# stevenknown/xpoly

Hardware: AMD Instinct MI355X
Metric: simplex pivots/sec (float tableau 4kx8k) (higher is better)
Workload: dtype f64; 1 GPU; dense LP m=4096 n=4095 (gen.hard_lp_f64: A~U(0.1,1), b=A x*, c=A^T y*), slack tableau 4096x8192 fp64 resident in HBM; one step = xpg_lp_begin (slack form rebuilt on the device) + 3840 pivots of the device-resident SIX::solveSlackForm loop = 120 full batches of 32; parallelism=replicas only (1 tableau per GPU)

## Files before the change

### xpoly_amd/csrc/ctx.hip.h

```cpp
#pragma once
#include <hip/hip_runtime.h>
#include <hip/hip_ext.h>
#include <map>
#include <mutex>
#include <string>
#include <utility>
#include <vector>
#include <stdio.h>
#include <stdlib.h>
#include <string.h>
#include "../../include/xpoly_amd.h"

namespace xpg { struct LoopState; }

struct xpg_ctx {
    int device;
    hipStream_t stream;
    std::string err;
    void * rowbuf; void * colbuf; xpg::LoopState * st; size_t row_cap, col_cap;
    void * stage; size_t stage_cap;
    void * hstage; size_t hstage_cap;
    void * hpack = 0; size_t hpack_cap = 0;
    void * hred = 0; size_t hred_cap = 0;
    std::vector<xpg_ctx *> lanes;
    std::vector<std::pair<void *, size_t> > dev_cache;
    size_t dev_cache_bytes = 0;
    void * slice_buf = 0; size_t slice_cap = 0;
    int loop_mode;
    int block_len;
    int loop_auto;
    int num_cus;
    int chain;
    int chain_local = 1;
    int chain_fold = 1;
    int chain_test_abort = 0;
    std::vector<hipEvent_t> ev0, ev1;
    int prof_cap, prof_n, prof_stride, prof_seen;
};

#define XPG_HIP(ctx, call)                                                         \
    do {                                                                           \
        hipError_t e_ = (call);                                                    \
        if (e_ != hipSuccess) {                                                    \
            (ctx)->err = std::string(#call) + ": " + hipGetErrorString(e_);        \
            return XPG_ERR_HIP;                                                    \
        }                                                                          \
    } while (0)

namespace xpg {

struct DeviceGuard {
    int prev = -1, mine = -1;
    explicit DeviceGuard(int device) : mine(device)
    {
        if (hipGetDevice(&prev) != hipSuccess) prev = -1;
        if (device >= 0 && prev != device) (void)hipSetDevice(device);
    }
    ~DeviceGuard() { if (prev >= 0 && mine >= 0 && prev != mine) (void)hipSetDevice(prev); }
    DeviceGuard(const DeviceGuard &) = delete;
    DeviceGuard & operator=(const DeviceGuard &) = delete;
};
#define XPG_BIND(ctx_) xpg::DeviceGuard xpg_bind_guard_((ctx_) ? (ctx_)->device : -1)

inline int round_up(int x, int a) { return (x + a - 1) / a * a; }

inline hipError_t lds_limit(const void * fn, int device, size_t bytes)
{
    static std::mutex mu;
    static std::map<std::pair<const void *, int>, size_t> cur;
    std::lock_guard<std::mutex> g(mu);
    size_t & c = cur[std::make_pair(fn, device)];
    if (bytes <= c) return hipSuccess;
    const hipError_t e = hipFuncSetAttribute(fn, hipFuncAttributeMaxDynamicSharedMemorySize, (int)bytes);
    if (e == hipSuccess) c = bytes;
    return e;
}

inline int pick_ld(int W)
{
    int ld = W % 16 == 0 ? W : round_up(W, 64);
    if (ld % 4112 == 0 || (ld + 16) % 4096 == 0) ld += 16;
    return ld;
}

struct DevBuf {
    void * p; size_t cap; xpg_ctx * owner;
    DevBuf() : p(0), cap(0), owner(0) {}
// ... 60 lines not shown
```

### xpoly_amd/csrc/lp_chain.hip.h

```cpp
#pragma once
#include "lp_blocked.hip.h"

namespace xpg {

enum { ST_CHAIN_STUCK = XPG_ERR_CHAIN_STUCK, CH_SPIN_LIMIT = 1 << 21, CH_CLOSE = 0x7FFFFFFF,
       CH_ARRIVE_TICKS = 30000,
       CH_VETO_TICKS = 100000,
       CH_GO = 1, CH_ABORT = 2 };
typedef unsigned int ch_u32x4 __attribute__((ext_vector_type(4)));

__device__ __forceinline__ unsigned long long ch_lo64(ch_u32x4 g) { return ((unsigned long long)g.y << 32) | g.x; }

__device__ __forceinline__ void ch_load_record(const void * p, ch_u32x4 (&g)[6])
{
    asm volatile("global_load_dwordx4 %0, %6, off sc1\n\t"
                 "global_load_dwordx4 %1, %6, off offset:16 sc1\n\t"
                 "global_load_dwordx4 %2, %6, off offset:32 sc1\n\t"
                 "global_load_dwordx4 %3, %6, off offset:48 sc1\n\t"
                 "global_load_dwordx4 %4, %6, off offset:64 sc1\n\t"
                 "global_load_dwordx4 %5, %6, off offset:80 sc1\n\t"
                 "s_waitcnt vmcnt(0)"
                 : "=&v"(g[0]), "=&v"(g[1]), "=&v"(g[2]), "=&v"(g[3]), "=&v"(g[4]), "=&v"(g[5]) : "v"(p) : "memory");
}
__device__ __forceinline__ void ch_load4(const void * p0, const void * p1, const void * p2, const void * p3,
// ... 110 lines not shown
{
    const unsigned lo = (unsigned)dpp_row_shr<CTRL>((int)(unsigned)x), hi = (unsigned)dpp_row_shr<CTRL>((int)(unsigned)(x >> 32));
    const unsigned long long t = ((unsigned long long)hi << 32) | lo;
    return t < x ? t : x;
}
__device__ __forceinline__ unsigned long long ch_wave_min_u64(unsigned long long x)
{
    x = ch_min_step<0x111>(x); x = ch_min_step<0x112>(x); x = ch_min_step<0x114>(x); x = ch_min_step<0x118>(x);
    const unsigned long long a = ch_readlane_u64(x, 15), b = ch_readlane_u64(x, 31), c = ch_readlane_u64(x, 47), d = ch_readlane_u64(x, 63);
    const unsigned long long ab = a < b ? a : b, cd = c < d ? c : d;
    return ab < cd ? ab : cd;
}

enum { CH_NAP_FROM = 96 };
#ifndef CH_POLL_NAP
#define CH_POLL_NAP 1
#endif
#ifndef CH_NAP_PICK
#define CH_NAP_PICK 32
#endif
#ifndef CH_NAP_PREP
#define CH_NAP_PREP 32
#endif

struct ChHist { double h[BLK_MAX]; };
__device__ __forceinline__ void ch_hist_load(ChHist & H, const double * hist)
{
#pragma unroll
    for (int s = 0; s < BLK_MAX; s++) H.h[s] = hist[64 * s];
}
template <bool STAR> __device__ __forceinline__ double ch_replay(double start, const ChHist & H, double cv, int t, int star)
{
    double a = start;
#pragma unroll
    for (int s = 0; s < BLK_MAX; s += 4) {
        if (s >= t) break;
        double p0 = H.h[s] * ch_readlane_f64(cv, s), p1 = H.h[s + 1] * ch_readlane_f64(cv, s + 1);
        double p2 = H.h[s + 2] * ch_readlane_f64(cv, s + 2), p3 = H.h[s + 3] * ch_readlane_f64(cv, s + 3);
        if (STAR) {
            const double ident = -0.0;
            p0 = s > star ? p0 : ident; p1 = s + 1 > star ? p1 : ident; p2 = s + 2 > star ? p2 : ident; p3 = s + 3 > star ? p3 : ident;
        }
        a = a + p0; a = a + p1; a = a + p2; a = a + p3;
    }
    return a;
}

struct ChWinner { int r, enter, leave, qstar, cc; uint32_t w; double a; unsigned long long cnv; };
enum { CH_CLOSE_ROW = 0x7FFFFFFE, CH_UNORDERED_ROW = 0x7FFFFFFD };

__device__ __forceinline__ char * ch_rec_g0(const LpView<F64> & v, int w) { return (char *)(v.blkR + BLK_REC_G0) + (size_t)w * 16; }
__device__ __forceinline__ char * ch_rec_pay(const LpView<F64> & v, int w) { return (char *)(v.blkR + BLK_REC_PAY) + (size_t)w * (BLK_REC_PAY_WORDS * 8); }
__device__ __forceinline__ char * ch_part_g0(const LpView<F64> & v, int w) { return (char *)v.blkP + (size_t)w * 16; }
__device__ __forceinline__ char * ch_part_pay(const LpView<F64> & v, int w) { return (char *)(v.blkP + BLK_PART_PAY) + (size_t)w * (BLK_PART_PAY_INTS * 4); }

__device__ __forceinline__ int ch_poll_records(const LpView<F64> & v, int npick, unsigned tag, int lane, ChWinner & W)
{
    const int nu = (npick + 63) >> 6;
    const int k0 = lane, k1 = lane + 64, k2 = lane + 128, k3 = lane + 192;
    const void * p0 = ch_rec_g0(v, k0 < npick ? k0 : k0 % npick);
    const void * p1 = ch_rec_g0(v, k1 < npick ? k1 : k0 % npick);
    const void * p2 = ch_rec_g0(v, k2 < npick ? k2 : k0 % npick);
    const void * p3 = ch_rec_g0(v, k3 < npick ? k3 : k0 % npick);
    ch_u32x4 g0, g1, g2, g3;
    unsigned spins = 0;
    for (;;) {
        bool ok;
        if (nu == 1) { g0 = ch_load1(p0); ok = g0.w == tag; }
        else { ch_load4(p0, p1, p2, p3, g0, g1, g2, g3); ok = g0.w == tag && g1.w == tag && g2.w == tag && g3.w == tag; }
        if (__all(ok)) break;
        if (++spins > CH_SPIN_LIMIT) return -3;
        __builtin_amdgcn_s_sleep(CH_POLL_NAP);
    }
    unsigned long long key = ~0ull; int row = INT_MAX, rec = 0;
    if (k0 < npick) { key = ch_lo64(g0); row = (int)g0.z; rec = k0; }
    if (nu > 1) {
        if (k1 < npick && ch_lo64(g1) < key) { key = ch_lo64(g1); row = (int)g1.z; rec = k1; }
        if (k2 < npick && ch_lo64(g2) < key) { key = ch_lo64(g2); row = (int)g2.z; rec = k2; }
        if (k3 < npick && ch_lo64(g3) < key) { key = ch_lo64(g3); row = (int)g3.z; rec = k3; }
    }
    if (__builtin_amdgcn_readfirstlane((int)g0.z) == CH_CLOSE_ROW) return -1;
    const unsigned long long kmin = ch_wave_min_u64(key);
    if (kmin == 0ull) return -1;
    if (kmin == ~0ull) return -2;
    const int myrow = key == kmin ? row : INT_MAX;
    W.r = wave_min_int(myrow);
    const unsigned long long hit = __ballot(myrow == W.r);
    return __builtin_amdgcn_readlane(rec, __ffsll((long long)hit) - 1);
}
__device__ __forceinline__ bool ch_load_winner(const LpView<F64> & v, int widx, unsigned tag, ChWinner & W)
{
    const char * p = ch_rec_pay(v, widx);
    ch_u32x4 g1, g2, g3;
    unsigned spins = 0;
    for (;;) {
        ch_load3(p, p + 16, p + 32, g1, g2, g3);
        if (__all(g1.w == tag && g2.w == tag && g3.w == tag)) break;
        if (++spins > CH_SPIN_LIMIT) return false;
        __builtin_amdgcn_s_sleep(CH_POLL_NAP);
    }
    W.a = __builtin_bit_cast(double, ch_lo64(g1)); W.leave = (int)g1.z;
    W.w = g2.x; W.cc = (int)g2.y; W.enter = (int)(g2.z & 0xFFFFFFu); W.qstar = (int)(g2.z >> 24) - 1;
    W.cnv = ch_lo64(g3);
    return true;
}

template <bool LOCAL> __device__ __forceinline__ void ch_commit_loop(const LpView<F64> & v, int batch, int t0, int B, int npick, int nprep,
                                                                     unsigned budget, unsigned done, unsigned tp, bool fold_next)
{
    LoopState * st = v.st;
    const int lane = (int)threadIdx.x;
    for (int t = t0; t < B; t++) {
        const unsigned tag = blk_epoch(batch, t);
        ChWinner g;
        const int widx = ch_poll_records(v, npick, tag, lane, g);
        if (widx == -3 || (widx >= 0 && !ch_load_winner(v, widx, tag, g))) { if (lane == 0) ch_st(&st->status, (int)ST_CHAIN_STUCK); return; }
        if (widx < 0) {
            if (lane == 0 && (widx == -2 || budget != 0)) st->blk.closed = 1;
            if (lane == 0 && t == 0) {
                st->blk.batch = batch; st->blk.n = 0; st->blk.closed = 1; st->blk.generic = 0;
                if (widx == -2) st->blk.want_generic = 1;
            }
            ch_drain();
            if (lane == 0)
                ch_store_granule<LOCAL>(ch_part_g0(v, nprep), (unsigned long long)(unsigned)INT_MAX, ((unsigned long long)(unsigned)CH_CLOSE_ROW << 32) | (unsigned long long)tag);
            return;
        }
        if (lane == 0) {
            const int enter = g.enter, leave = g.leave, r = g.r;
            if (!((g.w >> (leave & 31)) & 1u)) {
                ch_stl<LOCAL>(&v.ppt[(size_t)enter * v.pw + (leave >> 5)], g.w | (1u << (leave & 31)));
                if (LOCAL) ch_st_plain(&v.rowcnt[enter], ch_ld(&v.rowcnt[enter]) + 1);
                else __hip_atomic_fetch_add(&v.rowcnt[enter], 1, __ATOMIC_RELAXED, __HIP_MEMORY_SCOPE_AGENT);
                ch_stl<LOCAL>(&v.colcnt[leave], g.cc + 1);
            }
            ch_stl<LOCAL>(&v.nv[enter], (uint8_t)0); ch_stl<LOCAL>(&v.nv[leave], (uint8_t)1);
            ch_stl<LOCAL>(&v.bv[enter], (uint8_t)1); ch_stl<LOCAL>(&v.bv[leave], (uint8_t)0);
            ch_stl<LOCAL>(&v.eq2bv[r], enter); ch_stl<LOCAL>(&v.bv2eq[enter], r); ch_stl<LOCAL>(&v.bv2eq[leave], -1);
            if ((int)tp < v.trace_cap) { v.trace[2 * tp] = enter; v.trace[2 * tp + 1] = leave; }
            st->total_pivots = tp + 1;
            st->done = done + 1;
            st->blk.budget = budget - 1;
            if (t == 0) { st->blk.batch = batch; st->blk.closed = 0; st->blk.generic = 0; }
            st->blk.r[t] = r; st->blk.n = t + 1;
            st->blk.la_from_state = 0;
            st->blk.la_epoch = tag;
            if (t == B - 1 && fold_next) {
                for (int x = 0; x < 8; x++) st->blk.ch_arrive[x] = 0u;
                st->blk.ch_decide = 0u;
                st->blk.ch0_la_epoch = tag; st->blk.ch0_budget = budget - 1; st->blk.ch0_done = done + 1; st->blk.ch0_tp = tp + 1;
                st->blk.ch0_ticket = blk_ticket0(batch + 1);
            }
        }
        ch_drain();
        if (lane == 0)
            ch_store_granule<LOCAL>(ch_part_g0(v, nprep), (unsigned long long)(unsigned)INT_MAX, ((unsigned long long)(unsigned)g.r << 32) | (unsigned long long)tag);
        tp += 1; done += 1; budget -= 1;
    }
}

#ifdef XPG_STAMPS
__device__ unsigned long long g_ch_ts[4][BLK_MAX][8];
#define CH_TS(pt_) do { if (lane == 0 && tsw >= 0) g_ch_ts[tsw][t][pt_] = wall_clock64(); } while (0)
#else
#define CH_TS(pt_) do { } while (0)
#endif

inline int ch_hist_slots(int B, int line) { return line ? (B + 3) / 4 * 4 : BLK_MAX; }
inline size_t ch_lds_bytes(int B, int line)
{
    const size_t plain = (size_t)BLK_MAX * 64 * 8, with_line = (size_t)ch_hist_slots(B, line) * 64 * 8 + (size_t)line * 64 * 8;
    return line ? (with_line > plain ? with_line : plain) : plain;
}
template <bool LOCAL, int LINE>
__global__ __launch_bounds__(64) void k_blk_chain(LpView<F64> v, int batch, int t0, int B, int npick, int nprep, int nparts0, int force_abort, int fold_next)
{
    extern __shared__ __attribute__((aligned(16))) double ch_hist[];
    if (LOCAL && (blockIdx.x & 7u)) return;
    LoopState * st = v.st;
    const int w = LOCAL ? (int)(blockIdx.x >> 3) : (int)blockIdx.x, lane = (int)threadIdx.x;
    const unsigned nworkers = LOCAL ? gridDim.x >> 3 : gridDim.x;
    const bool fold = t0 == 0;
    if ((fold ? st->blk.ch0_ticket != blk_ticket0(batch) : st->blk.ch_epoch != blk_epoch(batch, t0 - 1)) ||
        st->status != ST_RUNNING || st->pricing != 0 || (fold && (st->blk.la_from_state != 0 || st->blk.want_generic != 0))) return;
    unsigned budget = fold ? st->blk.ch0_budget : st->blk.ch_budget, done = fold ? st->blk.ch0_done : st->blk.ch_done;
    const unsigned tp0 = fold ? st->blk.ch0_tp : st->blk.ch_tp;
    const unsigned la_tag = st->blk.ch0_la_epoch;
    const unsigned max_iter = st->max_iter;
    char * const decision = ch_part_g0(v, BLK_DECISION_SLOT);
    const unsigned roll_tag = fold ? blk_ticket0(batch) : blk_epoch(batch, t0 - 1);
    if (lane == 0) __hip_atomic_fetch_add(&st->blk.ch_arrive[LOCAL ? ch_xcc_id() : 0], 1u, __ATOMIC_RELAXED, __HIP_MEMORY_SCOPE_AGENT);
    if (w == (int)nworkers - 1) {
        const unsigned long long t_in = wall_clock64();
        bool go = false, misplaced = false;
        for (;;) {
#ifdef XPG_TEST_HOOKS
            if (force_abort) { misplaced = force_abort == 2; break; }
#endif
            const unsigned mine = ch_ld(&st->blk.ch_arrive[lane & 7]);
            unsigned sum = 0, top = 0;
#pragma unroll
            for (int x = 0; x < 8; x++) { const unsigned c = (unsigned)__builtin_amdgcn_readlane((int)mine, x); sum += c; top = c > top ? c : top; }
            if (top >= nworkers) { go = true; break; }
            if (sum >= nworkers) { misplaced = true; break; }
            if (wall_clock64() - t_in > (unsigned long long)CH_ARRIVE_TICKS) break;
            __builtin_amdgcn_s_sleep(CH_POLL_NAP);
        }
        unsigned prev = 0u;
        if (lane == 0) prev = atomicCAS(&st->blk.ch_decide, 0u, go ? (unsigned)CH_GO : (unsigned)CH_ABORT);
        prev = (unsigned)__builtin_amdgcn_readfirstlane((int)prev);
        if (prev != 0u) return;
        if (lane == 0) {
            if (go) { st->blk.ch_runs += 1u; if (fold) st->blk.ch_folds += 1u; }
            else { st->blk.closed = 1; st->blk.ch_aborts += 1u; if (misplaced) st->blk.ch_misplaced += 1u; }
        }
        ch_drain();
        if (lane == 0) ch_store_granule<false>(decision, (unsigned long long)(go ? CH_GO : CH_ABORT), (unsigned long long)roll_tag);
        if (go) ch_commit_loop<LOCAL>(v, batch, t0, B, npick, nprep, budget, done, tp0, fold_next != 0);
        return;
    }
    const int m = v.m, W = v.W, rhs = v.rhs, ld = v.ld, lim = v.rhs - 1;
    const bool picker = w < npick;
    const double * __restrict__ tab = (const double *)v.tab;
    double * K = (double *)v.blkK;
    double * E = (double *)v.blkE;
    double * const hist = ch_hist + lane;
    const int hslots = LINE ? (B + 3) / 4 * 4 : BLK_MAX;
    bool decided = false;
// ... 1 lines not shown
        if (decided) return true;
        unsigned spins = 0;
        const unsigned long long t_wait = wall_clock64();
        bool asked = false;
        for (;;) {
            const ch_u32x4 g = ch_load1(decision);
            if (g.z == roll_tag) { if (g.x != (unsigned)CH_GO) return false; decided = true; return true; }
            if (!asked && wall_clock64() - t_wait > (unsigned long long)CH_VETO_TICKS) {
                asked = true;
                unsigned prev = 0u;
                if (lane == 0) prev = atomicCAS(&st->blk.ch_decide, 0u, (unsigned)CH_ABORT);
                prev = (unsigned)__builtin_amdgcn_readfirstlane((int)prev);
                if (prev == 0u) {
                    if (lane == 0) { st->blk.closed = 1; st->blk.ch_aborts += 1u; }
                    ch_drain();
                    if (lane == 0) ch_store_granule<false>(decision, (unsigned long long)CH_ABORT, (unsigned long long)roll_tag);
                    return false;
                }
                if (prev == (unsigned)CH_ABORT) return false;
            }
            if (++spins > CH_SPIN_LIMIT) { if (lane == 0) ch_st(&st->status, (int)ST_CHAIN_STUCK); return false; }
            __builtin_amdgcn_s_sleep(CH_POLL_NAP);
        }
    };
#ifdef XPG_STAMPS
    const int tsw = w == 0 ? 0 : (w == npick - 1 ? 1 : (w == npick ? 2 : (w == npick + nprep - 1 ? 3 : -1)));
#endif

    const bool crowded = npick + nprep > CH_NAP_FROM;
    if (picker) {
        const int i = w * 64 + lane;
        const bool has_row = i < m;
        const int ic = has_row ? i : 0;
        for (int s = 0; s < hslots; s++) hist[64 * s] = 0.0;
        for (int s = 0; s < t0; s++) hist[64 * s] = has_row ? K[(size_t)ic * BLK_MAX + s] : 0.0;
        double * const lcache = ch_hist + (size_t)hslots * 64 + lane;
        int line_group = -1;
        int bi = v.eq2bv[ic];
        int sstar = -1;
        double bcur = tab[(size_t)ic * ld + rhs];
        double klast = 0.0;
        for (int s = 0; s < t0; s++) {
            const int rs = st->blk.r[s];
            if (rs == i) sstar = s;
            const double ks = has_row ? K[(size_t)ic * BLK_MAX + s] : 0.0;
            if (s + 1 < t0) {
                const double eb = E[(size_t)s * ld + rhs];
                const double pb = ks * eb;
                bcur = (rs == i) ? eb : (bcur + pb);
            } else klast = ks;
        }
        int r_prev = t0 > 0 ? st->blk.r[t0 - 1] : -1;
        int first_prev = -1;
#pragma unroll 1
        for (int t = t0; t < B; t++) {
            const unsigned want_part = t > 0 ? blk_epoch(batch, t - 1) : la_tag, tag = blk_epoch(batch, t);
            CH_TS(0);
            ChHist H;
            ch_hist_load(H, hist);
            if (CH_NAP_PICK && crowded && t > t0) __builtin_amdgcn_s_sleep(CH_NAP_PICK);
            const int cnt = t == t0 ? nparts0 : nprep;
            const int lo = t == t0 ? 1 : 0;
            int nf = INT_MAX;
            for (int base = 0; base <= cnt; base += 256) {
                const int span = cnt + 1 - base;
                auto slot = [&](int k) -> const void * {
                    int kk = k <= cnt ? k : base + (lane % span);
                    kk = kk < lo ? lo : kk;
                    return ch_part_g0(v, kk == 0 ? nprep : kk - 1);
                };
                const void * p0 = slot(base + lane);
                const void * p1 = slot(base + lane + 64);
                const void * p2 = slot(base + lane + 128);
                const void * p3 = slot(base + lane + 192);
                ch_u32x4 g0, g1, g2, g3;
                unsigned spins = 0;
                for (;;) {
                    ch_load4(p0, p1, p2, p3, g0, g1, g2, g3);
                    const bool ok = g0.z == want_part && g1.z == want_part && g2.z == want_part && g3.z == want_part;
                    if (__all(ok)) break;
                    if (base == 0 && lo == 0 && (unsigned)__builtin_amdgcn_readfirstlane((int)g0.z) == want_part
                        && __builtin_amdgcn_readfirstlane((int)g0.w) == CH_CLOSE_ROW) return;
                    if (++spins > CH_SPIN_LIMIT) { if (lane == 0) ch_st(&st->status, (int)ST_CHAIN_STUCK); return; }
                    __builtin_amdgcn_s_sleep(CH_POLL_NAP);
                }
                nf = min(min(nf, (int)g0.x), min(min((int)g1.x, (int)g2.x), (int)g3.x));
                if (base == 0 && lo == 0) {
                    r_prev = __builtin_amdgcn_readfirstlane((int)g0.w);
                    if (r_prev == CH_CLOSE_ROW) return;
                    if (i == r_prev) { bi = first_prev; sstar = t - 1; }
                }
            }
            CH_TS(1);
            const int first = wave_min_int(nf);
            const bool fast = first >= 0 && first < rhs && done < max_iter && budget != 0;
            if (!fast) {
                if (!wait_decision()) return;
                if (lane == 0) ch_store_granule3<LOCAL>(ch_rec_g0(v, w), ~0u, ~0u, (unsigned)CH_CLOSE_ROW, tag);
                return;
            }
            double x0_mem = 0.0;
            constexpr int LN = LINE ? LINE : 16;
            double2 lnew[LN / 2];
            const bool line_miss = LINE && first / LN != line_group;
            if (!LINE) x0_mem = tab[(size_t)ic * ld + first];
            else if (line_miss) {
                const double2 * lp2 = (const double2 *)&tab[(size_t)ic * ld + (size_t)(first / LN) * LN];
#pragma unroll
                for (int q = 0; q < LN / 2; q++) lnew[q] = lp2[q];
            }
            const uint32_t pw_word = ch_ld(&v.ppt[(size_t)first * v.pw + (bi >> 5)]);
            const int cc = ch_ld(&v.colcnt[bi]);
            const double ev_mem = ch_ld(&E[(size_t)(lane + 1 < t ? lane : 0) * ld + first]);
            const double c0_mem = v.obj[first].v;
            double ev = 0.0;
            if (t == 0) {
                if (lane == 33) ev = c0_mem;
            } else {
                const bool fresh = lane >= 32 && lane <= 34;
                const char * gp = ch_part_pay(v, (lane == 34 ? rhs : first) >> 6) + (fresh ? 16 * (lane - 32) : 0);
                unsigned spins = 0;
                for (;;) {
                    const ch_u32x4 g = ch_load1(gp);
                    if (__all(g.z == want_part || !fresh)) { if (fresh) ev = __builtin_bit_cast(double, ch_lo64(g)); break; }
                    if (++spins > CH_SPIN_LIMIT) { if (lane == 0) ch_st(&st->status, (int)ST_CHAIN_STUCK); return; }
                    __builtin_amdgcn_s_sleep(CH_POLL_NAP);
                }
            }
            CH_TS(2);
            if (lane + 1 < t) ev = ev_mem;
            if (LINE && line_miss) {
#pragma unroll
                for (int q = 0; q < LN / 2; q++) { lcache[64 * (2 * q)] = lnew[q].x; lcache[64 * (2 * q + 1)] = lnew[q].y; }
                line_group = first / LN;
            }
            const double x0 = LINE ? lcache[64 * (first % LN)] : x0_mem;
            const double ec_new = ch_readlane_f64(ev, 32), eb_new = ch_readlane_f64(ev, 34);
            const unsigned long long cnv_bits = __builtin_bit_cast(unsigned long long, ch_readlane_f64(ev, 33));
            if (lane == t - 1) ev = ec_new;
            if (lane >= t) ev = -1.0;
            if (t > 0) {
                const double pb = klast * eb_new;
                bcur = (i == r_prev) ? eb_new : (bcur + pb);
            }
            double a;
            if (__any(sstar >= 0)) {
                const double es = __shfl(ev, sstar >= 0 ? sstar : 0);
                a = ch_replay<true>(sstar >= 0 ? es : x0, H, ev, t, sstar);
            } else a = ch_replay<false>(x0, H, ev, t, -1);
            CH_TS(5);
            klast = -a;
            hist[64 * t] = klast;
            if (!wait_decision()) return;
            if (has_row) ch_stl<LOCAL>(&K[(size_t)i * BLK_MAX + t], klast);
            unsigned long long key = ~0ull;
            bool unordered = false;
            if (has_row && !le(F64(a), zero<F64>()) && !((pw_word >> (bi & 31)) & 1u) && cc < lim) {
                const double q = bcur / a;
                unordered = q != q;
                key = ch_ratio_key(q);
            }
            if (__any(unordered)) {
                if (lane == 0) ch_store_granule3<LOCAL>(ch_rec_g0(v, w), 0u, 0u, (unsigned)CH_UNORDERED_ROW, tag);
                key = ~0ull;
            }
            const bool told = __any(unordered);
            CH_TS(6);
            const unsigned long long kmin = ch_wave_min_u64(key);
            const unsigned long long hit = __ballot(key == kmin);
            const bool publisher = kmin != ~0ull ? (lane == __ffsll((long long)hit) - 1) : (lane == 0);
            CH_TS(7);
            if (publisher && !told) {
                ch_store_granule3<LOCAL>(ch_rec_g0(v, w), (unsigned)kmin, (unsigned)(kmin >> 32), (unsigned)(kmin != ~0ull ? i : INT_MAX), tag);
                const unsigned long long ab = to_bits(F64(a));
                char * pay = ch_rec_pay(v, w);
                ch_store_granule3<LOCAL>(pay, (unsigned)ab, (unsigned)(ab >> 32), (unsigned)bi, tag);
                ch_store_granule3<LOCAL>(pay + 16, pw_word, (unsigned)cc, (unsigned)first | ((unsigned)(sstar + 1) << 24), tag);
                ch_store_granule3<LOCAL>(pay + 32, (unsigned)cnv_bits, (unsigned)(cnv_bits >> 32), 0u, tag);
            }
            CH_TS(3);
            first_prev = first;
            done += 1; budget -= 1;
        }
        return;
    }

    const int wp = w - npick;
    const int j = wp * 64 + lane;
    const bool has_col = j < W;
    const int jc = has_col ? j : 0;
    for (int s = 0; s < hslots; s++) hist[64 * s] = 0.0;
    for (int s = 0; s < t0; s++) hist[64 * s] = has_col ? E[(size_t)s * ld + jc] : 0.0;
    F64 oj = has_col ? v.obj[jc] : zero<F64>();
    if (!wait_decision()) return;
#pragma unroll 1
    for (int t = t0; t < B; t++) {
        const unsigned tag = blk_epoch(batch, t);
        CH_TS(0);
        ChHist H;
        ch_hist_load(H, hist);
        if (CH_NAP_PREP && crowded && t > t0) __builtin_amdgcn_s_sleep(CH_NAP_PREP);
        ChWinner g;
        const int widx = ch_poll_records(v, npick, tag, lane, g);
        if (widx == -3) { if (lane == 0) ch_st(&st->status, (int)ST_CHAIN_STUCK); return; }
        if (widx < 0) return;
        CH_TS(4);
        const int r = g.r;
        const double x0 = tab[(size_t)r * ld + jc];
        const bool in_vars = has_col && j < rhs;
        const int nv_mem = (int)ch_ld(&v.nv[in_vars ? jc : 0]), rc_mem = ch_ld(&v.rowcnt[in_vars ? jc : 0]);
        const double kv_mem = ch_ld(&K[(size_t)r * BLK_MAX + (lane < t ? lane : 0)]);
        if (!ch_load_winner(v, widx, tag, g)) { if (lane == 0) ch_st(&st->status, (int)ST_CHAIN_STUCK); return; }
        const int nvj = in_vars ? nv_mem : 0, rcj0 = in_vars ? rc_mem : INT_MAX;
        const double kv = lane < t ? kv_mem : -1.0;
        CH_TS(1);
        const int enter = g.enter, leave = g.leave;
        const F64 sc = div(one<F64>(), F64(g.a));
        const int smode = scale_mode(sc);
        const F64 cnv = from_bits<F64>(g.cnv);
        const int cmode = scale_mode(cnv);
        const int qstar = __builtin_amdgcn_readfirstlane(g.qstar);
        const double x = qstar >= 0 ? ch_replay<true>(hist[64 * qstar], H, kv, t, qstar) : ch_replay<false>(x0, H, kv, t, -1);
        CH_TS(2);
        const F64 e = scaled(F64(x), sc, smode);
        hist[64 * t] = e.v;
        CH_TS(5);
        int nf = INT_MAX, any = 0;
        if (has_col) {
            ch_stl<LOCAL>(&E[(size_t)t * ld + j], e.v);
            F64 tt = mul(e, minus_one<F64>());
            if (j >= rhs) tt = neg(tt);
            tt = scaled(tt, cnv, cmode);
            const bool in = j < rhs;
            const bool nv_mem = in && j != enter && j != leave && nvj != 0;
            const bool nv_old = in && (j == enter ? true : (j == leave ? false : nv_mem));
            const bool nv_new = in && (j == enter ? false : (j == leave ? true : nv_mem));
            const int rcj = (in && j != enter) ? rcj0 : INT_MAX;
            if (j < enter && in && !nv_old) oj = zero<F64>();
            oj = add(tt, oj);
            v.obj[j] = oj;
            if (nv_new && gt(oj, zero<F64>())) { any = 1; if (rcj < lim) nf = j; }
        }
        CH_TS(3);
        nf = wave_min_int(nf);
        any = __ballot(any != 0) != 0ull ? 1 : 0;
        char * pay = ch_part_pay(v, wp);
        if (has_col && j == nf) {
            ch_store_granule<LOCAL>(pay, to_bits(e), (unsigned long long)tag);
            ch_store_granule<LOCAL>(pay + 16, to_bits(oj), (unsigned long long)tag);
        }
        if (has_col && j == rhs) ch_store_granule<LOCAL>(pay + 32, to_bits(e), (unsigned long long)tag);
        if (lane == 0) ch_store_granule<LOCAL>(ch_part_g0(v, wp), ((unsigned long long)(unsigned)any << 32) | (unsigned)nf, (unsigned long long)tag);
        CH_TS(6);
    }
}

}
```

### xpoly_amd/csrc/lp_host.hip.h

```cpp
#pragma once
#include <hip/hip_runtime.h>
#include <hip/hip_ext.h>
#include <map>
#include <mutex>
#include <string>
#include <type_traits>
#include <utility>
#include <vector>
#include <stdio.h>
#include "../../include/xpoly_amd.h"
#include "ctx.hip.h"
#include "lp_kernels.hip.h"
#include "lp_blocked.hip.h"
#include "lp_chain.hip.h"

namespace xpg {

template <class S> inline void launch_update(xpg_ctx * ctx, const LpView<S> & v, int guarded);
inline bool prof_open(xpg_ctx * ctx)
{
    if (ctx->prof_n >= ctx->prof_cap) return false;
    if ((ctx->prof_seen++ % ctx->prof_stride) != 0) return false;
    (void)hipEventRecord(ctx->ev0[ctx->prof_n], ctx->stream);
    return true;
// ... 46 lines not shown
inline bool blk_shape_ok(int W) { return (W + 255) / 256 <= 510; }
inline bool chain_shape_ok(const xpg_ctx * ctx, int m, int W)
{
    const int cpick = (m + 63) / 64, cprep = (W + 63) / 64;
    const int cus = ctx->num_cus > 0 ? ctx->num_cus : 1;
    return cpick <= BLK_REC_MAX && cprep <= 510 && cpick + cprep + 1 <= 8 * cus;
}
struct BlkPlan {
    bool chain;
    bool local;
    int line;
    int cpick, cprep, workers;
    size_t lds;
    int sweep_rows;
};
inline BlkPlan blk_plan(const xpg_ctx * ctx, int m, int W, int ld, int B, bool ref_pricing, bool chain_off, bool chain_spread, bool fold)
{
    BlkPlan p;
    p.cpick = (m + 63) / 64; p.cprep = (W + 63) / 64; p.workers = p.cpick + p.cprep + 1;
    const int cus = ctx->num_cus > 0 ? ctx->num_cus : 1;
    p.chain = ctx->chain && !chain_off && ref_pricing && (B > 1 || fold) && chain_shape_ok(ctx, m, W);
    p.local = p.chain && ctx->chain_local && !chain_spread && p.workers <= (cus / 8) * 9;
    static const int line_env = [] { const char * s = xpg_hook("XPG_CHAIN_LINE"); return s ? atoi(s) : -1; }();
    auto line_fits = [&](int cols) {
        return (size_t)p.workers * ch_lds_bytes(B, cols) <= (size_t)(cus / 8) * 160 * 1024 &&
               (size_t)p.workers <= (size_t)(cus / 8) * ((size_t)160 * 1024 / ch_lds_bytes(B, cols));
    };
    const bool want_line = p.local && (line_env == 1 || line_env == 8 || (line_env != 0 && ld % 512 == 0));
    p.line = !want_line ? 0 : (line_env != 8 && line_fits(16)) ? 16 : line_fits(8) ? 8 : 0;
    p.lds = ch_lds_bytes(B, p.line);
    p.sweep_rows = (size_t)m * ld * sizeof(double) > ((size_t)320 << 20) ? 32 : 16;
    return p;
}
template <class S> inline void launch_blk_batch(xpg_ctx *, const LpView<S> &, int, int, bool, bool, bool, bool, bool, bool) {}
template <> inline void launch_blk_batch<F64>(xpg_ctx * ctx, const LpView<F64> & v, int batch, int B, bool ref_pricing, bool closes_often, bool chain_off,
                                              bool chain_spread, bool fold, bool next_folds)
{
    const int strips = (v.W + 511) / 512;
    const int tq = (v.W + 63) / 64 <= 510 ? 64 : 256, tp = 64;
    const int want_pick = (v.m + tp - 1) / tp;
    const int npick = want_pick < BLK_PICK_WGS ? want_pick : BLK_PICK_WGS;
    const dim3 gprep((v.W + tq - 1) / tq);
    const BlkPlan pl = blk_plan(ctx, v.m, v.W, v.ld, B, ref_pricing, chain_off, chain_spread, fold);
    const int cpick = pl.cpick, cprep = pl.cprep, workers = pl.workers;
    for (int t = 0; t < B; t++) {
        if (pl.chain && (t == 1 || fold)) {
            const int t0 = fold ? 0 : 1;
            const int test_abort = ctx->chain_test_abort;
            const bool local = pl.local;
            const int fa = test_abort > 0 ? (batch % test_abort == test_abort - 1 ? 1 : 0)
                                          : (test_abort < 0 && local && batch % -test_abort == -test_abort - 1 ? 2 : 0);
            const int nparts0 = (int)gprep.x;
            const int fn = next_folds ? 1 : 0;
            const int line = pl.line;
            const size_t lds = pl.lds;
            if (local && line == 16) hipLaunchKernelGGL((k_blk_chain<true, 16>), dim3(8 * workers), dim3(64), lds, ctx->stream, v, batch, t0, B, cpick, cprep, nparts0, fa, fn);
            else if (local && line == 8) hipLaunchKernelGGL((k_blk_chain<true, 8>), dim3(8 * workers), dim3(64), lds, ctx->stream, v, batch, t0, B, cpick, cprep, nparts0, fa, fn);
            else if (local) hipLaunchKernelGGL((k_blk_chain<true, 0>), dim3(8 * workers), dim3(64), lds, ctx->stream, v, batch, t0, B, cpick, cprep, nparts0, fa, fn);
            else hipLaunchKernelGGL((k_blk_chain<false, 0>), dim3(workers), dim3(64), lds, ctx->stream, v, batch, t0, B, cpick, cprep, nparts0, fa, fn);
            break;
        }
        hipLaunchKernelGGL(k_blk_pick, dim3(npick), dim3(tp), 0, ctx->stream, v, batch, t, (int)gprep.x);
        if (t == 0) hipLaunchKernelGGL(k_blk_pick_generic, dim3(1), dim3(1024), 0, ctx->stream, v, batch, (int)gprep.x);
        hipLaunchKernelGGL(k_blk_prep, gprep, dim3(tq), 0, ctx->stream, v, batch, t);
    }
    const bool timed = B == ctx->block_len && ctx->prof_n < ctx->prof_cap && (ctx->prof_seen++ % ctx->prof_stride) == 0;
    hipEvent_t e0 = timed ? ctx->ev0[ctx->prof_n] : nullptr, e1 = timed ? ctx->ev1[ctx->prof_n] : nullptr;
#define XPG_BLK_LAUNCH(ROWS_, UNR_, CAP_)                                                                                 \
    hipExtLaunchKernelGGL((k_blk_sweep<ROWS_, UNR_, CAP_>), dim3(strips, (v.m + ROWS_ - 1) / ROWS_), dim3(256), 0,        \
                          ctx->stream, e0, e1, 0, (double *)v.tab, v.m, v.W, v.ld, (const double *)v.blkE,                \
                          (const double *)v.blkK, v.st, batch, 0, ctx->block_len)
#define XPG_BLK_FULL(ROWS_, UNR_, NB_)                                                                                    \
    hipExtLaunchKernelGGL((k_blk_sweep_full<ROWS_, UNR_, NB_>), dim3(blk_sweep_grid(strips, (v.m + ROWS_ - 1) / ROWS_)), \
                          dim3(256), 0, ctx->stream, e0, e1, 0, (double *)v.tab, v.m, v.W, v.ld,                          \
                          (const double *)v.blkE, (const double *)v.blkK, v.st, batch, closes_often ? 1 : 0,              \
                          batch & 1, ctx->block_len)
    const bool full = B == 32 || B == 24 || B == 16;
    if (B == 32 && pl.sweep_rows == 32) XPG_BLK_FULL(32, 2, 32);
    else if (B == 32) XPG_BLK_FULL(16, 2, 32);
    else if (B == 24) XPG_BLK_FULL(16, 2, 24);
    else if (B == 16) XPG_BLK_FULL(16, 4, 16);
    else if (B <= 8) XPG_BLK_LAUNCH(32, 8, 8);
    else XPG_BLK_LAUNCH(32, 4, 16);
    if (closes_often && full)
        hipLaunchKernelGGL((k_blk_sweep<32, 4, 16>), dim3(strips, (v.m + 31) / 32), dim3(256), 0, ctx->stream, (double *)v.tab,
                           v.m, v.W, v.ld, (const double *)v.blkE, (const double *)v.blkK, v.st, batch, B, ctx->block_len);
#undef XPG_BLK_LAUNCH
#undef XPG_BLK_FULL
    if (timed) ctx->prof_n++;
}
template <> inline void launch_update<R32>(xpg_ctx * ctx, const LpView<R32> & v, int guarded)
{
    const bool timed = prof_open(ctx);
    hipLaunchKernelGGL((k_update_r32<1>), dim3(v.m, (v.W + 255) / 256), dim3(256), 0, ctx->stream, v, guarded);
    if (timed) prof_close(ctx);
}

struct LpBase {
    virtual ~LpBase() {}
    xpg_ctx * ctx;
    int kind;
};

template <class S> struct Lp : LpBase {
    LpView<S> v;
    int n0;
    int m;
    S * d_leq; S * d_tgtf;
    S * d_maxv;
    std::vector<void *> owned;
    size_t tab_elems;
    int ld_cap = 0;
// ... 397 lines not shown
```

### xpoly_amd/csrc/xpoly_amd.hip

```cpp
#include <hip/hip_runtime.h>
#include <stdlib.h>
#include <string.h>
#include <atomic>
#include <new>
#include <map>
#include <algorithm>
#include <thread>
#include <vector>
#include "../../include/xpoly_amd.h"
#ifndef XPG_PART
#define XPG_PART (-1)
#endif
#define XPG_IN(p_) (XPG_PART < 0 || XPG_PART == (p_))
#include "scalar.hip.h"
#include "ctx.hip.h"
#if XPG_IN(0)
#include "lp_kernels.hip.h"
#include "lp_pipe_r32.hip.h"
#include "lp_fused_r32.hip.h"
#include "lp_host.hip.h"
#include "warm_mip.hip.h"
#include "warm_mip_batch.hip.h"
#endif
#if XPG_IN(1) || XPG_IN(2)
// ... 13 lines not shown
namespace xpg {
extern template int batch_dev<F64>(xpg_ctx *, int, int, const F64 *, const F64 *, int, int, unsigned, int32_t *, F64 *, F64 *, uint32_t *, int);
extern template int batch_dev<R32>(xpg_ctx *, int, int, const R32 *, const R32 *, int, int, unsigned, int32_t *, R32 *, R32 *, uint32_t *, int);
}
#elif XPG_PART == 1
namespace xpg {
template int batch_dev<F64>(xpg_ctx *, int, int, const F64 *, const F64 *, int, int, unsigned, int32_t *, F64 *, F64 *, uint32_t *, int);
template int batch_dev<R32>(xpg_ctx *, int, int, const R32 *, const R32 *, int, int, unsigned, int32_t *, R32 *, R32 *, uint32_t *, int);
}
#endif

static_assert(sizeof(F64) == 8 && sizeof(R32) == 8, "both scalars are 8 bytes");
static_assert(sizeof(xpg_rat32) == sizeof(R32), "ABI layout of a rational");

#if XPG_IN(0)
struct xpg_lp { LpBase * impl; };

extern "C" {

const char * xpg_version(void) { return "xpoly_amd 0.1 (gfx950)"; }

int xpg_device_count(void)
{
    int n = 0;
    if (hipGetDeviceCount(&n) != hipSuccess) return 0;
    return n;
}

int xpg_create(xpg_ctx ** out, int device)
{
    if (!out) return XPG_ERR_SHAPE;
    *out = 0;
    int n = 0;
    if (hipGetDeviceCount(&n) != hipSuccess || n <= 0 || device < 0 || device >= n)
        return XPG_ERR_NO_DEVICE;
    xpg::DeviceGuard bind(device);
    xpg_ctx * c = new (std::nothrow) xpg_ctx();
    if (!c) return XPG_ERR_ALLOC;
    c->device = device;
    c->rowbuf = c->colbuf = 0; c->st = 0; c->row_cap = c->col_cap = 0;
    c->stage = 0; c->stage_cap = 0;
    c->hstage = 0; c->hstage_cap = 0;
    const char * lm = xpg_env("XPG_LOOP");
    if (lm && lm[0] == 's') lm = nullptr;
    c->loop_mode = lm && lm[0] == 'b' ? 3 : 0;
    const char * ch = xpg_env("XPG_CHAIN");
    c->chain = ch ? atoi(ch) : 1;
    const char * cx = xpg_hook("XPG_CHAIN_XCD");
    c->chain_local = cx ? (atoi(cx) != 0 ? 1 : 0) : 1;
    const char * cf = xpg_hook("XPG_CHAIN_FOLD");
    c->chain_fold = cf ? (atoi(cf) != 0 ? 1 : 0) : 1;
    const char * cta = xpg_hook("XPG_CHAIN_TEST_ABORT");
    c->chain_test_abort = cta ? atoi(cta) : 0;
    c->num_cus = 0;
    if (hipDeviceGetAttribute(&c->num_cus, hipDeviceAttributeMultiprocessorCount, device) != hipSuccess) c->num_cus = 0;
    c->loop_auto = lm ? 0 : 1;
    const char * bl = xpg_env("XPG_BLOCK");
    c->block_len = bl ? atoi(bl) : BLK_DEFAULT;
    if (c->block_len < 1) c->block_len = 1;
    if (c->block_len > BLK_MAX) c->block_len = BLK_MAX;
    c->prof_cap = 0; c->prof_n = 0; c->prof_stride = 1; c->prof_seen = 0;
    if (hipStreamCreateWithFlags(&c->stream, hipStreamNonBlocking) != hipSuccess) { delete c; return XPG_ERR_HIP; }
    if (hipMalloc((void **)&c->st, sizeof(LoopState)) != hipSuccess) { (void)hipStreamDestroy(c->stream); delete c; return XPG_ERR_ALLOC; }
    *out = c;
    return 0;
}

void xpg_destroy(xpg_ctx * ctx)
{
    if (!ctx) return;
    XPG_BIND(ctx);
    (void)hipStreamSynchronize(ctx->stream);
    for (hipEvent_t e : ctx->ev0) (void)hipEventDestroy(e);
    for (hipEvent_t e : ctx->ev1) (void)hipEventDestroy(e);
    if (ctx->rowbuf) (void)hipFree(ctx->rowbuf);
    if (ctx->colbuf) (void)hipFree(ctx->colbuf);
    if (ctx->st) (void)hipFree(ctx->st);
    if (ctx->stage) (void)hipFree(ctx->stage);
    if (ctx->hstage) (void)hipHostFree(ctx->hstage);
    if (ctx->hpack) (void)hipHostFree(ctx->hpack);
    if (ctx->hred) (void)hipHostFree(ctx->hred);
    if (ctx->slice_buf) (void)hipFree(ctx->slice_buf);
    for (xpg_ctx * l : ctx->lanes) xpg_destroy(l);
    ctx->lanes.clear();
    for (auto & b : ctx->dev_cache) (void)hipFree(b.first);
    (void)hipStreamDestroy(ctx->stream);
    delete ctx;
}

int xpg_profile_begin(xpg_ctx * ctx, int cap, int stride)
{
    XPG_BIND(ctx);
    if (!ctx || cap < 0 || stride < 1) return XPG_ERR_SHAPE;
    XPG_HIP(ctx, hipStreamSynchronize(ctx->stream));
    while ((int)ctx->ev0.size() < cap) {
        hipEvent_t a, b;
        XPG_HIP(ctx, hipEventCreate(&a));
        XPG_HIP(ctx, hipEventCreate(&b));
        ctx->ev0.push_back(a); ctx->ev1.push_back(b);
    }
    ctx->prof_cap = cap; ctx->prof_n = 0; ctx->prof_stride = stride; ctx->prof_seen = 0;
    return 0;
}

int xpg_profile_end(xpg_ctx * ctx, int * launches, double * total_ms)
{
// ... 330 lines not shown
    if (chain_off) *chain_off = p->chain_off ? 1 : 0;
    if (runs) *runs = hs.blk.ch_runs;
    return 0;
}

int xpg_lp_loop_info(xpg_lp * lp, int32_t * out, int n)
{
    if (!lp || !lp->impl || !out || n < 0) return XPG_ERR_SHAPE;
    int32_t f[10] = {0, 0, 0, 0, 0, 0, 0, 0, 0, 0};
    if (lp->impl->kind == 0) ((Lp<F64> *)lp->impl)->loop_info(f);
    else ((Lp<R32> *)lp->impl)->loop_info(f);
    for (int k = 0; k < n && k < 10; k++) out[k] = f[k];
    return 0;
}

#ifdef XPG_STAMPS
int xpg_lp_debug(xpg_lp * lp, unsigned long long * out8)
{
    if (!lp || !lp->impl) return XPG_ERR_SHAPE;
    LoopState hs;
    int rc = lp->impl->kind == 0 ? ((Lp<F64> *)lp->impl)->read_state(&hs) : ((Lp<R32> *)lp->impl)->read_state(&hs);
    if (rc) return rc;
    for (int k = 0; k < 8; k++) out8[k] = hs.blk.dbg[k];
    return 0;
}
int xpg_lp_debug_staged(xpg_lp * lp, double * E, double * K, int * ld, int * blk_max, int cap)
{
    if (!lp || !lp->impl || lp->impl->kind != 0) return XPG_ERR_SHAPE;
    Lp<F64> * p = (Lp<F64> *)lp->impl;
    xpg_ctx * ctx = p->ctx;
    if (ld) *ld = p->v.ld;
    if (blk_max) *blk_max = BLK_MAX;
    if ((E || K) && cap != BLK_MAX) return XPG_ERR_SHAPE;
    if (E) XPG_HIP(ctx, hipMemcpy(E, p->v.blkE, (size_t)BLK_MAX * p->v.ld * 8, hipMemcpyDeviceToHost));
    if (K) XPG_HIP(ctx, hipMemcpy(K, p->v.blkK, (size_t)p->v.m * BLK_MAX * 8, hipMemcpyDeviceToHost));
    return 0;
}
int xpg_lp_debug_counts(xpg_lp * lp, int * rowcnt, int * colcnt, int n)
{
    if (!lp || !lp->impl || lp->impl->kind != 0) return XPG_ERR_SHAPE;
    Lp<F64> * p = (Lp<F64> *)lp->impl;
    xpg_ctx * ctx = p->ctx;
    XPG_HIP(ctx, hipMemcpy(rowcnt, p->v.rowcnt, (size_t)n * 4, hipMemcpyDeviceToHost));
    XPG_HIP(ctx, hipMemcpy(colcnt, p->v.colcnt, (size_t)n * 4, hipMemcpyDeviceToHost));
    return 0;
}
int xpg_lp_debug_chain_ts(xpg_lp * lp, unsigned long long * out, int * blk_max, int cap)
{
    if (!lp || !lp->impl) return XPG_ERR_SHAPE;
    xpg_ctx * ctx = lp->impl->ctx;
    if (blk_max) *blk_max = BLK_MAX;
    if (!out) return 0;
    if (cap != BLK_MAX) return XPG_ERR_SHAPE;
    XPG_HIP(ctx, hipMemcpyFromSymbol(out, HIP_SYMBOL(g_ch_ts), sizeof(unsigned long long) * 4 * BLK_MAX * 8));
    return 0;
}
int xpg_lp_debug_rows(xpg_lp * lp, double * out)
{
    if (!lp || !lp->impl) return XPG_ERR_SHAPE;
    xpg_ctx * ctx = lp->impl->ctx;
    XPG_HIP(ctx, hipMemcpyFromSymbol(out, HIP_SYMBOL(g_dbg_rows), sizeof(double) * 4 * 8192));
    return 0;
}
#endif

int xpg_lp_chain_folds(xpg_lp * lp, unsigned * folds)
{
    if (!lp || !lp->impl || !folds) return XPG_ERR_SHAPE;
    XPG_BIND(lp->impl->ctx);
    *folds = 0;
    if (lp->impl->kind != 0) return 0;
    LoopState hs;
    const int rc = ((Lp<F64> *)lp->impl)->read_state(&hs);
    if (rc) return rc;
    *folds = hs.blk.ch_folds;
    return 0;
}

int xpg_lp_trace(xpg_lp * lp, int32_t * pairs, int cap_pairs, int * n_pairs)
{
    if (!lp || !lp->impl || !n_pairs) return XPG_ERR_SHAPE;
    xpg_ctx * ctx = lp->impl->ctx;
    XPG_BIND(ctx);
    LoopState hs;
    int rc; int * d_trace; int cap;
    if (lp->impl->kind == 0) { Lp<F64> * p = (Lp<F64> *)lp->impl; rc = p->read_state(&hs); d_trace = p->v.trace; cap = p->v.trace_cap; }
    else { Lp<R32> * p = (Lp<R32> *)lp->impl; rc = p->read_state(&hs); d_trace = p->v.trace; cap = p->v.trace_cap; }
    if (rc) return rc;
    int n = (int)hs.total_pivots;
    *n_pairs = n;
    if (n > cap) n = cap;
    if (n > cap_pairs) n = cap_pairs;
    if (pairs && n > 0) {
        XPG_HIP(ctx, hipMemcpyAsync(pairs, d_trace, (size_t)n * 8, hipMemcpyDeviceToHost, ctx->stream));
        XPG_HIP(ctx, hipStreamSynchronize(ctx->stream));
    }
    return 0;
}

int xpg_trim(xpg_ctx * ctx)
{
    XPG_BIND(ctx);
    if (!ctx) return XPG_ERR_SHAPE;
    XPG_HIP(ctx, hipStreamSynchronize(ctx->stream));
    for (auto & b : ctx->dev_cache) (void)hipFree(b.first);
    ctx->dev_cache.clear(); ctx->dev_cache_bytes = 0;
    if (ctx->hpack) { (void)hipHostFree(ctx->hpack); ctx->hpack = 0; ctx->hpack_cap = 0; }
// ... 714 lines not shown
```

Before: 135,600 pivots/s.

## Early-exit chain pick wait once lowest-index entering-column partial is known

In the device-resident chain kernel, the per-step wait for all column-pick partials now proceeds as soon as the lowest tagged partial with a valid candidate is found and every lower slot is tagged, instead of waiting for all partials and doing a wave min. The full tag check is deferred until just before the ratio-test record is published, so the row update overlaps the stragglers. The K history store is moved after publication. It also adds test hooks and extra timestamp points. The risk is extra polling loads and subtle ordering correctness with late partials.

```diff
diff --git a/xpoly_amd/csrc/ctx.hip.h b/xpoly_amd/csrc/ctx.hip.h
--- a/xpoly_amd/csrc/ctx.hip.h
+++ b/xpoly_amd/csrc/ctx.hip.h
@@ -33,6 +33,7 @@
     int chain;
     int chain_local = 1;
     int chain_fold = 1;
+    int chain_test_late_from = -1;
     int chain_test_abort = 0;
     std::vector<hipEvent_t> ev0, ev1;
     int prof_cap, prof_n, prof_stride, prof_seen;
diff --git a/xpoly_amd/csrc/lp_chain.hip.h b/xpoly_amd/csrc/lp_chain.hip.h
--- a/xpoly_amd/csrc/lp_chain.hip.h
+++ b/xpoly_amd/csrc/lp_chain.hip.h
@@ -186,6 +186,7 @@
 __device__ __forceinline__ char * ch_rec_g0(const LpView<F64> & v, int w) { return (char *)(v.blkR + BLK_REC_G0) + (size_t)w * 16; }
 __device__ __forceinline__ char * ch_rec_pay(const LpView<F64> & v, int w) { return (char *)(v.blkR + BLK_REC_PAY) + (size_t)w * (BLK_REC_PAY_WORDS * 8); }
 __device__ __forceinline__ char * ch_part_g0(const LpView<F64> & v, int w) { return (char *)v.blkP + (size_t)w * 16; }
+__device__ __forceinline__ const unsigned * ch_part_tag(const LpView<F64> & v, int w) { return (const unsigned *)ch_part_g0(v, w) + 2; }
 __device__ __forceinline__ char * ch_part_pay(const LpView<F64> & v, int w) { return (char *)(v.blkP + BLK_PART_PAY) + (size_t)w * (BLK_PART_PAY_INTS * 4); }
 
 __device__ __forceinline__ int ch_poll_records(const LpView<F64> & v, int npick, unsigned tag, int lane, ChWinner & W)
@@ -237,6 +238,13 @@
     W.w = g2.x; W.cc = (int)g2.y; W.enter = (int)(g2.z & 0xFFFFFFu); W.qstar = (int)(g2.z >> 24) - 1;
     W.cnv = ch_lo64(g3);
     return true;
+}
+
+__device__ __forceinline__ int ch_needed_lane(unsigned long long tagged, unsigned long long cand)
+{
+    if (!cand) return 0;
+    const int l = __ffsll((long long)cand) - 1;
+    return (~tagged & ((1ull << l) - 1ull)) == 0ull ? l : 0;
 }
 
 template <bool LOCAL> __device__ __forceinline__ void ch_commit_loop(const LpView<F64> & v, int batch, int t0, int B, int npick, int nprep,
@@ -294,10 +302,13 @@
 }
 
 #ifdef XPG_STAMPS
-__device__ unsigned long long g_ch_ts[4][BLK_MAX][8];
+enum { CH_TS_POINTS = 16 };
+__device__ unsigned long long g_ch_ts[4][BLK_MAX][CH_TS_POINTS];
 #define CH_TS(pt_) do { if (lane == 0 && tsw >= 0) g_ch_ts[tsw][t][pt_] = wall_clock64(); } while (0)
+#define CH_TS_VAL(pt_, x_) do { if (lane == 0 && tsw >= 0) g_ch_ts[tsw][t][pt_] = (unsigned long long)(x_); } while (0)
 #else
 #define CH_TS(pt_) do { } while (0)
+#define CH_TS_VAL(pt_, x_) do { } while (0)
 #endif
 
 inline int ch_hist_slots(int B, int line) { return line ? (B + 3) / 4 * 4 : BLK_MAX; }
@@ -307,7 +318,7 @@
     return line ? (with_line > plain ? with_line : plain) : plain;
 }
 template <bool LOCAL, int LINE>
-__global__ __launch_bounds__(64) void k_blk_chain(LpView<F64> v, int batch, int t0, int B, int npick, int nprep, int nparts0, int force_abort, int fold_next)
+__global__ __launch_bounds__(64) void k_blk_chain(LpView<F64> v, int batch, int t0, int B, int npick, int nprep, int nparts0, int force_abort, int fold_next, int late_from)
 {
     extern __shared__ __attribute__((aligned(16))) double ch_hist[];
     if (LOCAL && (blockIdx.x & 7u)) return;
@@ -415,6 +426,8 @@
         }
         int r_prev = t0 > 0 ? st->blk.r[t0 - 1] : -1;
         int first_prev = -1;
+        auto slot_of = [&](int k) { const int kk = k <= nprep ? k : lane % (nprep + 1); return kk == 0 ? nprep : kk - 1; };
+        const int ai0 = slot_of(lane), ai1 = slot_of(lane + 64), ai2 = slot_of(lane + 128), ai3 = slot_of(lane + 192);
 #pragma unroll 1
         for (int t = t0; t < B; t++) {
             const unsigned want_part = t > 0 ? blk_epoch(batch, t - 1) : la_tag, tag = blk_epoch(batch, t);
@@ -424,18 +437,49 @@
             if (CH_NAP_PICK && crowded && t > t0) __builtin_amdgcn_s_sleep(CH_NAP_PICK);
             const int cnt = t == t0 ? nparts0 : nprep;
             const int lo = t == t0 ? 1 : 0;
+            auto slot = [&](int base, int k) -> const void * {
+                int kk = k <= cnt ? k : base + (lane % (cnt + 1 - base));
+                kk = kk < lo ? lo : kk;
+                return ch_part_g0(v, kk == 0 ? nprep : kk - 1);
+            };
             int nf = INT_MAX;
-            for (int base = 0; base <= cnt; base += 256) {
-                const int span = cnt + 1 - base;
-                auto slot = [&](int k) -> const void * {
-                    int kk = k <= cnt ? k : base + (lane % span);
-                    kk = kk < lo ? lo : kk;
-                    return ch_part_g0(v, kk == 0 ? nprep : kk - 1);
-                };
-                const void * p0 = slot(base + lane);
-                const void * p1 = slot(base + lane + 64);
-                const void * p2 = slot(base + lane + 128);
-                const void * p3 = slot(base + lane + 192);
+            bool early = false;
+            if (t > t0 && cnt < 256 && done < max_iter && budget != 0) {
+                const void * p0 = ch_part_g0(v, ai0);
+                const unsigned long long real = cnt >= 63 ? ~0ull : (1ull << (cnt + 1)) - 1ull;
+                unsigned spins = 0;
+#ifdef XPG_STAMPS
+                unsigned long long ts_a = 0;
+#endif
+                for (;;) {
+                    const ch_u32x4 g = ch_load1(p0);
+                    const unsigned long long tg = __ballot(g.z == want_part) & real;
+                    const unsigned long long cd = __ballot(g.z == want_part && (int)g.x != INT_MAX) & real;
+                    if (tg & 1ull) {
+#ifdef XPG_STAMPS
+                        if (!ts_a) ts_a = wall_clock64();
+#endif
+                        if (__builtin_amdgcn_readfirstlane((int)g.w) == CH_CLOSE_ROW) return;
+                    }
+                    const int l = ch_needed_lane(tg, cd);
+                    if (l > 0) {
+                        nf = __builtin_amdgcn_readlane((int)g.x, l);
+                        r_prev = __builtin_amdgcn_readfirstlane((int)g.w);
+                        early = true;
+                        CH_TS_VAL(8, ts_a); CH_TS_VAL(11, l);
+                        break;
+                    }
+                    if (tg == real) break;
+                    if (++spins > CH_SPIN_LIMIT) { if (lane == 0) ch_st(&st->status, (int)ST_CHAIN_STUCK); return; }
+                    __builtin_amdgcn_s_sleep(CH_POLL_NAP);
+                }
+                if (early && i == r_prev) { bi = first_prev; sstar = t - 1; }
+            }
+            if (!early) for (int base = 0; base <= cnt; base += 256) {
+                const void * p0 = slot(base, base + lane);
+                const void * p1 = slot(base, base + lane + 64);
+                const void * p2 = slot(base, base + lane + 128);
+                const void * p3 = slot(base, base + lane + 192);
                 ch_u32x4 g0, g1, g2, g3;
                 unsigned spins = 0;
                 for (;;) {
@@ -452,10 +496,11 @@
                     r_prev = __builtin_amdgcn_readfirstlane((int)g0.w);
                     if (r_prev == CH_CLOSE_ROW) return;
                     if (i == r_prev) { bi = first_prev; sstar = t - 1; }
+                    CH_TS(8); CH_TS_VAL(11, cnt + 1);
                 }
             }
             CH_TS(1);
-            const int first = wave_min_int(nf);
+            const int first = early ? nf : wave_min_int(nf);
             const bool fast = first >= 0 && first < rhs && done < max_iter && budget != 0;
             if (!fast) {
                 if (!wait_decision()) return;
@@ -498,6 +543,13 @@
                 line_group = first / LN;
             }
             const double x0 = LINE ? lcache[64 * (first % LN)] : x0_mem;
+            unsigned all0 = want_part, all1 = want_part, all2 = want_part, all3 = want_part;
+            asm volatile("" :: "v"(ev_mem), "v"(c0_mem), "v"(pw_word), "v"(cc), "v"(x0_mem));
+            if (early) {
+                all0 = ch_ld(ch_part_tag(v, ai0)); all1 = ch_ld(ch_part_tag(v, ai1));
+                all2 = ch_ld(ch_part_tag(v, ai2)); all3 = ch_ld(ch_part_tag(v, ai3));
+                CH_TS(13);
+            }
             const double ec_new = ch_readlane_f64(ev, 32), eb_new = ch_readlane_f64(ev, 34);
             const unsigned long long cnv_bits = __builtin_bit_cast(unsigned long long, ch_readlane_f64(ev, 33));
             if (lane == t - 1) ev = ec_new;
@@ -515,7 +567,6 @@
             klast = -a;
             hist[64 * t] = klast;
             if (!wait_decision()) return;
-            if (has_row) ch_stl<LOCAL>(&K[(size_t)i * BLK_MAX + t], klast);
             unsigned long long key = ~0ull;
             bool unordered = false;
             if (has_row && !le(F64(a), zero<F64>()) && !((pw_word >> (bi & 31)) & 1u) && cc < lim) {
@@ -523,17 +574,27 @@
                 unordered = q != q;
                 key = ch_ratio_key(q);
             }
-            if (__any(unordered)) {
-                if (lane == 0) ch_store_granule3<LOCAL>(ch_rec_g0(v, w), 0u, 0u, (unsigned)CH_UNORDERED_ROW, tag);
-                key = ~0ull;
-            }
             const bool told = __any(unordered);
+            if (told) key = ~0ull;
             CH_TS(6);
             const unsigned long long kmin = ch_wave_min_u64(key);
             const unsigned long long hit = __ballot(key == kmin);
             const bool publisher = kmin != ~0ull ? (lane == __ffsll((long long)hit) - 1) : (lane == 0);
             CH_TS(7);
-            if (publisher && !told) {
+            if (early) {
+                unsigned rounds = 0;
+                while (!__all(all0 == want_part && all1 == want_part && all2 == want_part && all3 == want_part)) {
+                    if (++rounds > CH_SPIN_LIMIT) { if (lane == 0) ch_st(&st->status, (int)ST_CHAIN_STUCK); return; }
+                    __builtin_amdgcn_s_sleep(CH_POLL_NAP);
+                    ch_u32x4 g0, g1, g2, g3;
+                    ch_load4(ch_part_g0(v, ai0), ch_part_g0(v, ai1), ch_part_g0(v, ai2), ch_part_g0(v, ai3), g0, g1, g2, g3);
+                    all0 = g0.z; all1 = g1.z; all2 = g2.z; all3 = g3.z;
+                }
+                CH_TS(10); CH_TS_VAL(12, rounds);
+            }
+            if (told) {
+                if (lane == 0) ch_store_granule3<LOCAL>(ch_rec_g0(v, w), 0u, 0u, (unsigned)CH_UNORDERED_ROW, tag);
+            } else if (publisher) {
                 ch_store_granule3<LOCAL>(ch_rec_g0(v, w), (unsigned)kmin, (unsigned)(kmin >> 32), (unsigned)(kmin != ~0ull ? i : INT_MAX), tag);
                 const unsigned long long ab = to_bits(F64(a));
                 char * pay = ch_rec_pay(v, w);
@@ -542,6 +603,7 @@
                 ch_store_granule3<LOCAL>(pay + 32, (unsigned)cnv_bits, (unsigned)(cnv_bits >> 32), 0u, tag);
             }
             CH_TS(3);
+            if (has_row) ch_stl<LOCAL>(&K[(size_t)i * BLK_MAX + t], klast);
             first_prev = first;
             done += 1; budget -= 1;
         }
@@ -608,6 +670,9 @@
         nf = wave_min_int(nf);
         any = __ballot(any != 0) != 0ull ? 1 : 0;
         char * pay = ch_part_pay(v, wp);
+#ifdef XPG_TEST_HOOKS
+        if (late_from >= 0 && wp >= late_from) __builtin_amdgcn_s_sleep(127);
+#endif
         if (has_col && j == nf) {
             ch_store_granule<LOCAL>(pay, to_bits(e), (unsigned long long)tag);
             ch_store_granule<LOCAL>(pay + 16, to_bits(oj), (unsigned long long)tag);
diff --git a/xpoly_amd/csrc/lp_host.hip.h b/xpoly_amd/csrc/lp_host.hip.h
--- a/xpoly_amd/csrc/lp_host.hip.h
+++ b/xpoly_amd/csrc/lp_host.hip.h
@@ -122,12 +122,13 @@
                                           : (test_abort < 0 && local && batch % -test_abort == -test_abort - 1 ? 2 : 0);
             const int nparts0 = (int)gprep.x;
             const int fn = next_folds ? 1 : 0;
+            const int lf = ctx->chain_test_late_from;
             const int line = pl.line;
             const size_t lds = pl.lds;
-            if (local && line == 16) hipLaunchKernelGGL((k_blk_chain<true, 16>), dim3(8 * workers), dim3(64), lds, ctx->stream, v, batch, t0, B, cpick, cprep, nparts0, fa, fn);
-            else if (local && line == 8) hipLaunchKernelGGL((k_blk_chain<true, 8>), dim3(8 * workers), dim3(64), lds, ctx->stream, v, batch, t0, B, cpick, cprep, nparts0, fa, fn);
-            else if (local) hipLaunchKernelGGL((k_blk_chain<true, 0>), dim3(8 * workers), dim3(64), lds, ctx->stream, v, batch, t0, B, cpick, cprep, nparts0, fa, fn);
-            else hipLaunchKernelGGL((k_blk_chain<false, 0>), dim3(workers), dim3(64), lds, ctx->stream, v, batch, t0, B, cpick, cprep, nparts0, fa, fn);
+            if (local && line == 16) hipLaunchKernelGGL((k_blk_chain<true, 16>), dim3(8 * workers), dim3(64), lds, ctx->stream, v, batch, t0, B, cpick, cprep, nparts0, fa, fn, lf);
+            else if (local && line == 8) hipLaunchKernelGGL((k_blk_chain<true, 8>), dim3(8 * workers), dim3(64), lds, ctx->stream, v, batch, t0, B, cpick, cprep, nparts0, fa, fn, lf);
+            else if (local) hipLaunchKernelGGL((k_blk_chain<true, 0>), dim3(8 * workers), dim3(64), lds, ctx->stream, v, batch, t0, B, cpick, cprep, nparts0, fa, fn, lf);
+            else hipLaunchKernelGGL((k_blk_chain<false, 0>), dim3(workers), dim3(64), lds, ctx->stream, v, batch, t0, B, cpick, cprep, nparts0, fa, fn, lf);
             break;
         }
         hipLaunchKernelGGL(k_blk_pick, dim3(npick), dim3(tp), 0, ctx->stream, v, batch, t, (int)gprep.x);
diff --git a/xpoly_amd/csrc/xpoly_amd.hip b/xpoly_amd/csrc/xpoly_amd.hip
--- a/xpoly_amd/csrc/xpoly_amd.hip
+++ b/xpoly_amd/csrc/xpoly_amd.hip
@@ -89,6 +89,8 @@
     c->chain_fold = cf ? (atoi(cf) != 0 ? 1 : 0) : 1;
     const char * cta = xpg_hook("XPG_CHAIN_TEST_ABORT");
     c->chain_test_abort = cta ? atoi(cta) : 0;
+    const char * clf = xpg_hook("XPG_CHAIN_TEST_LATE_FROM");
+    c->chain_test_late_from = clf ? atoi(clf) : -1;
     c->num_cus = 0;
     if (hipDeviceGetAttribute(&c->num_cus, hipDeviceAttributeMultiprocessorCount, device) != hipSuccess) c->num_cus = 0;
     c->loop_auto = lm ? 0 : 1;
@@ -525,7 +527,7 @@
     if (blk_max) *blk_max = BLK_MAX;
     if (!out) return 0;
     if (cap != BLK_MAX) return XPG_ERR_SHAPE;
-    XPG_HIP(ctx, hipMemcpyFromSymbol(out, HIP_SYMBOL(g_ch_ts), sizeof(unsigned long long) * 4 * BLK_MAX * 8));
+    XPG_HIP(ctx, hipMemcpyFromSymbol(out, HIP_SYMBOL(g_ch_ts), sizeof(unsigned long long) * 4 * BLK_MAX * CH_TS_POINTS));
     return 0;
 }
 int xpg_lp_debug_rows(xpg_lp * lp, double * out)
```

Measured after the change: 132,700 pivots/s, median of 2. -2.1%, worse.
